# analysiscenter/pydens

Measured on NVIDIA H100. Metric: collocation points/sec (fit step), higher is better.
Workload: dtype f32

## Files before the change

__graft_entry__.py:

```python
import concurrent.futures
import os
import subprocess
import sys

ROOT = os.path.dirname(os.path.abspath(__file__))
CSRC = os.path.join(ROOT, 'pydens_b200', 'csrc')
BUILD = os.path.join(ROOT, 'build')
LIB = os.path.join(ROOT, 'pydens_b200', 'libpinn_b200.so')
EMUL_SRC = os.path.join(ROOT, 'tests', 'emul', 'pinn_emul.cpp')
EMUL_LIB = os.path.join(ROOT, 'tests', 'emul', 'libpinn_emul.so')

NVCC_FLAGS = ['-gencode', 'arch=compute_90a,code=sm_90a', '-lineinfo', '-O3', '-std=c++17',
              '-Xcompiler', '-fPIC', '-I', os.path.join(ROOT, 'include')]
UNITS = ([('step_gen', 4, 3, 4), ('step_gen', 4, 0, 2), ('step_gen', 3, 2, 3), ('step_gen', 3, 0, 1)]
         + [('step', n, 0, n) for n in (4, 3)]
         + [('step_gen', n, 0, n) for n in (2, 1, 0)] + [('step', n, 0, n) for n in (2, 1, 0)]
         + [('step_gmem', n, n, n) for n in (6, 5)] + [('hi_jet', n, 3, 4) for n in (4, 3, 2, 1)]
         + [('wide', n, 0, n) for n in (4, 3, 2, 1, 0)] + [('small', n, 0, n) for n in (4, 3, 2, 1, 0)])
HEADERS = ['pinn_device.cuh', 'pinn_step_kernel.cuh', 'pinn_wide_kernel.cuh', 'pinn_small_kernel.cuh', 'pinn_host_plan.h',
           'pinn_device_hi.cuh', 'pinn_hi_kernel.cuh', os.path.join(ROOT, 'include', 'pinn_b200.h')]


def _mtime(path):
    return os.path.getmtime(path) if os.path.exists(path) else 0.0


def _nvcc():
    for cand in (os.environ.get('NVCC'), '/usr/local/cuda/bin/nvcc', 'nvcc'):
        if cand and (os.path.isabs(cand) and os.path.exists(cand) or not os.path.isabs(cand)):
            return cand
    return 'nvcc'


def _compile_one(unit):
    if isinstance(unit, str):
        src, name, defines = unit, os.path.splitext(unit)[0], []
    else:
        family, nf, lo, hi = unit
        src, name = 'pinn_instances.cu', 'pinn_%s_nf%d_%d-%d' % (family, nf, lo, hi)
        defines = ['-DPINN_UNIT=PINN_%s' % family.upper(), '-DPINN_NF=%d' % nf, '-DPINN_LO=%d' % lo, '-DPINN_HI=%d' % hi]
    obj = os.path.join(BUILD, name + '.o')
    srcp = os.path.join(CSRC, src)
    newest = max([_mtime(srcp)] + [_mtime(h if os.path.isabs(h) else os.path.join(CSRC, h)) for h in HEADERS])
    if _mtime(obj) >= newest:
        return obj, ''
    cmd = [_nvcc()] + NVCC_FLAGS + defines + ['-Xptxas', '-v', '-c', srcp, '-o', obj]
    res = subprocess.run(cmd, capture_output=True, text=True)
    if res.returncode != 0:
        raise RuntimeError('nvcc failed for %s:\n%s\n%s' % (name, res.stdout, res.stderr))
    return obj, res.stderr


def build(verbose=False, force=False):
# ... 66 lines not shown
```

pydens_b200/csrc/pinn_device.cuh:

```cuda
#pragma once

#include <stdint.h>
#include <math.h>
#include "../../include/pinn_b200.h"

#if defined(__CUDACC__)
#define PINN_HD __host__ __device__ __forceinline__
#define PINN_D  __device__ __forceinline__
#else
#define PINN_HD inline
#define PINN_D  inline
struct float4 { float x, y, z, w; };
struct float2 { float x, y; };
inline float2 make_float2(float x, float y) { float2 r; r.x = x; r.y = y; return r; }
#endif

#ifndef PINN_UNR_WIDE
#define PINN_UNR_WIDE 4
#endif
#ifndef PINN_BWD_UNR_WIDE
#define PINN_BWD_UNR_WIDE 1
#endif

#define PINN_FFMA2(a2, s, c2) make_float2(fmaf((a2).x, (s), (c2).x), fmaf((a2).y, (s), (c2).y))
#define PINN_FMUL2(a2, s)     make_float2((a2).x * (s), (a2).y * (s))
#define PINN_FFMA2V(a2, b2, c2) make_float2(fmaf((a2).x, (b2).x, (c2).x), fmaf((a2).y, (b2).y, (c2).y))
#define PINN_FMUL2V(a2, b2)     make_float2((a2).x * (b2).x, (a2).y * (b2).y)

namespace pinn {

struct DevLayer {
    int n_in, n_out, act;
    int w_off, b_off;
    int wt_s;
    int w_s;
    int b_s;
    int n_out_p4, n_in_p8;
    int unit_base;
    int post_base;
// ... 221 lines not shown
    const float2 out = PINN_FFMA2(t, k.p, make_float2(k.r, k.r));
    return k.ident ? z : out;
}

PINN_HD ActD act_from_stored(const ActC& k, float a) {
    ActD r;
    if (k.zs) { act_terms_z(k.zs, a, r.a, r.s1, r.s2, r.s3); return r; }
    r.a = a;
    r.s1 = fmaf(fmaf(k.c2, a, k.c1), a, k.c0);
    r.s2 = r.s1 * fmaf(k.d1, a, k.d0);
    r.s3 = r.s1 * fmaf(fmaf(k.e2, a, k.e1), a, k.e0);
    return r;
}

template <int NF, int NS, bool GEN = true>
PINN_HD void load_post_jet(const float* __restrict__ row, int RS, const ActC& k, float (&a)[1 + NF + NS]) {
    float av = row[0];
    float s1 = fmaf(fmaf(k.c2, av, k.c1), av, k.c0);
    float s2 = s1 * fmaf(k.d1, av, k.d0);
    if (GEN && k.zs) { float s3; act_terms_z(k.zs, row[0], av, s1, s2, s3); }
    a[0] = av;
#pragma unroll
    for (int d = 0; d < NF; ++d) {
        float zd = row[(1 + d) * RS];
        a[1 + d] = s1 * zd;
        if (d < NS) {
            float zdd = row[(1 + NF + d) * RS];
            a[1 + NF + d] = fmaf(s2 * zd, zd, s1 * zdd);
        }
    }
}

template <int NF, int NS, bool GEN = true>
PINN_HD void load_post_jet2(const float* __restrict__ rowa, const float* __restrict__ rowb, int RS, const ActC& k,
                            float2 (&a)[1 + NF + NS]) {
    float2 av = make_float2(rowa[0], rowb[0]);
    float2 s1 = PINN_FFMA2V(PINN_FFMA2(av, k.c2, make_float2(k.c1, k.c1)), av, make_float2(k.c0, k.c0));
    float2 s2 = PINN_FMUL2V(s1, PINN_FFMA2(av, k.d1, make_float2(k.d0, k.d0)));
    if (GEN && k.zs) {
        float s3;
        const float za = av.x, zb = av.y;
        act_terms_z(k.zs, za, av.x, s1.x, s2.x, s3);
        act_terms_z(k.zs, zb, av.y, s1.y, s2.y, s3);
    }
    a[0] = av;
#pragma unroll
    for (int d = 0; d < NF; ++d) {
        const float2 zd = make_float2(rowa[(1 + d) * RS], rowb[(1 + d) * RS]);
        a[1 + d] = PINN_FMUL2V(s1, zd);
        if (d < NS) {
            const float2 zdd = make_float2(rowa[(1 + NF + d) * RS], rowb[(1 + NF + d) * RS]);
            a[1 + NF + d] = PINN_FFMA2V(PINN_FMUL2V(s2, zd), zd, PINN_FMUL2V(s1, zdd));
        }
    }
}

template <int NF, int NS, int NB, bool GEN = true>
PINN_HD void fwd_block_hidden(const float* __restrict__ Wt, int wt_stride, const float* __restrict__ bias,
                              int n_in, const float* __restrict__ in_rows, int RS, const ActC& in_act,
                              float2 (&acc)[NB * 2][1 + NF + NS]) {
    constexpr int C = 1 + NF + NS;
#pragma unroll
    for (int j = 0; j < NB * 2; ++j) {
        acc[j][0] = make_float2(bias[2 * j], bias[2 * j + 1]);
#pragma unroll
        for (int c = 1; c < C; ++c) acc[j][c] = make_float2(0.0f, 0.0f);
    }
    constexpr int UNR = (C >= 8) ? PINN_UNR_WIDE : ((C >= 6) ? 2 : 1);
#pragma unroll UNR
    for (int k = 0; k < n_in; ++k) {
        float a[C];
        load_post_jet<NF, NS, GEN>(in_rows + (size_t)k * C * RS, RS, in_act, a);
        const float4* wrow = reinterpret_cast<const float4*>(Wt + (size_t)k * wt_stride);
#pragma unroll
        for (int g = 0; g < NB; ++g) {
            const float4 w = wrow[g];
            const float2 w01 = make_float2(w.x, w.y), w23 = make_float2(w.z, w.w);
#pragma unroll
            for (int c = 0; c < C; ++c) {
                acc[2 * g + 0][c] = PINN_FFMA2(w01, a[c], acc[2 * g + 0][c]);
                acc[2 * g + 1][c] = PINN_FFMA2(w23, a[c], acc[2 * g + 1][c]);
            }
        }
    }
}

template <int NF, int NS, int NB>
PINN_HD void fwd_block_input(const float* __restrict__ Wt, int wt_stride, const float* __restrict__ bias,
                             int n_in, const float* __restrict__ coords, int RS, const float* __restrict__ dirv,
                             float2 (&acc)[NB * 2][1 + NF + NS]) {
    constexpr int C = 1 + NF + NS;
#pragma unroll
    for (int j = 0; j < NB * 2; ++j) {
        acc[j][0] = make_float2(bias[2 * j], bias[2 * j + 1]);
#pragma unroll
        for (int c = 1; c < C; ++c) acc[j][c] = make_float2(0.0f, 0.0f);
    }
#pragma unroll 1
    for (int k = 0; k < n_in; ++k) {
        float x = coords[(size_t)k * RS];
        float vd[NF > 0 ? NF : 1];
#pragma unroll
        for (int d = 0; d < NF; ++d) vd[d] = dirv[d * PINN_MAX_DIMS + k];
        const float4* wrow = reinterpret_cast<const float4*>(Wt + (size_t)k * wt_stride);
#pragma unroll
        for (int g = 0; g < NB; ++g) {
            const float4 w = wrow[g];
            const float2 w01 = make_float2(w.x, w.y), w23 = make_float2(w.z, w.w);
            acc[2 * g + 0][0] = PINN_FFMA2(w01, x, acc[2 * g + 0][0]);
            acc[2 * g + 1][0] = PINN_FFMA2(w23, x, acc[2 * g + 1][0]);
#pragma unroll
            for (int d = 0; d < NF; ++d) {
                acc[2 * g + 0][1 + d] = PINN_FFMA2(w01, vd[d], acc[2 * g + 0][1 + d]);
                acc[2 * g + 1][1 + d] = PINN_FFMA2(w23, vd[d], acc[2 * g + 1][1 + d]);
            }
        }
    }
}

template <int NF, int NS, int NB, bool GEN = true>
PINN_HD void store_block(float* __restrict__ out_rows, int RS, const ActC& act, int j0, int n_out,
                         const float2 (&acc)[NB * 2][1 + NF + NS]) {
    constexpr int C = 1 + NF + NS;
#pragma unroll
    for (int h = 0; h < NB * 2; ++h) {
        const float2 a = act_store2<GEN>(act, acc[h][0]);
#pragma unroll
        for (int q = 0; q < 2; ++q) {
            const int j = 2 * h + q;
            const bool ok = j0 + j < n_out;
            float* row = out_rows + (size_t)(ok ? j0 + j : j0) * C * RS;
            if (ok) row[0] = q ? a.y : a.x;
#pragma unroll
            for (int c = 1; c < C; ++c)
                if (ok) row[(size_t)c * RS] = q ? acc[h][c].y : acc[h][c].x;
        }
    }
}

template <int NF, int NS, int JF, bool GEN = true>
PINN_HD void fwd_layer(const DevLayer& L, const float* __restrict__ sw, const float* __restrict__ in_rows,
                       bool in_is_coords, int in_act_id, const float* __restrict__ dirv,
                       float* __restrict__ out_rows, int RS) {
    constexpr int NBMAX = JF / 4;
    const float* Wt = sw + L.wt_s;
    const float* bias = sw + L.b_s;
    const ActC in_act = make_actc(in_act_id);
    const ActC out_act = make_actc(L.act);
#pragma unroll 1
    for (int j0 = 0; j0 < L.n_out; j0 += JF) {
        int nb = (L.n_out_p4 - j0) / 4;
        if (nb > NBMAX) nb = NBMAX;
#define PINN_FWD_CASE(NB)                                                                           \
        {                                                                                           \
            float2 acc[NB * 2][1 + NF + NS];                                                        \
            if (in_is_coords)                                                                       \
                fwd_block_input<NF, NS, NB>(Wt + j0, L.n_out_p4, bias + j0, L.n_in, in_rows, RS,    \
                                            dirv, acc);                                             \
            else                                                                                    \
                fwd_block_hidden<NF, NS, NB, GEN>(Wt + j0, L.n_out_p4, bias + j0, L.n_in, in_rows, RS,   \
                                             in_act, acc);                                          \
            store_block<NF, NS, NB, GEN>(out_rows, RS, out_act, j0, L.n_out, acc);                    \
        }
        if (NBMAX >= 4 && nb == 4) PINN_FWD_CASE(4)
        else if (NBMAX >= 3 && nb == 3) PINN_FWD_CASE(3)
        else if (NBMAX >= 2 && nb == 2) PINN_FWD_CASE(2)
        else PINN_FWD_CASE(1)
#undef PINN_FWD_CASE
    }
}

template <bool GEN = true>
PINN_HD const float* layer_output(const DevPlan& P, int p, const float* __restrict__ units, int C, int RS,
                                  int& act_id) {
    const DevLayer& Lp = P.layer[p];
    if (GEN && Lp.post_base >= 0) { act_id = PINN_ACT_NONE; return units + (size_t)Lp.post_base * C * RS; }
    act_id = Lp.act;
    return units + (size_t)Lp.unit_base * C * RS;
}

template <int NF, int NS>
PINN_HD void skip_sum_pass(const DevPlan& P, int l, float* __restrict__ units, int RS) {
    constexpr int C = 1 + NF + NS;
    const DevLayer& L = P.layer[l];
    const ActC own = make_actc(L.act);
    int src_act;
    const float* src_rows = layer_output(P, L.skip_src, units, C, RS, src_act);
    const ActC srcc = make_actc(src_act);
    const float* pre_rows = units + (size_t)L.unit_base * C * RS;
    float* post_rows = units + (size_t)L.post_base * C * RS;
#pragma unroll 1
    for (int j = 0; j < L.n_out; ++j) {
        float a[C], b[C];
        load_post_jet<NF, NS>(pre_rows + (size_t)j * C * RS, RS, own, a);
        load_post_jet<NF, NS>(src_rows + (size_t)j * C * RS, RS, srcc, b);
#pragma unroll
        for (int c = 0; c < C; ++c) post_rows[((size_t)j * C + c) * RS] = a[c] + b[c];
    }
}

template <int NF, int NS, bool GEN = true>
PINN_HD void fwd_final(const DevLayer& L, const float* __restrict__ sw, const float* __restrict__ in_rows,
                       bool in_is_coords, int in_act_id, const float* __restrict__ dirv, int RS,
                       float (&N)[1 + NF + NS]) {
    constexpr int C = 1 + NF + NS;
    const ActC in_act = make_actc(in_act_id);
    const float* w = sw + L.w_s;
    N[0] = sw[L.b_s];
#pragma unroll
    for (int c = 1; c < C; ++c) N[c] = 0.0f;
    if (in_is_coords) {
        for (int k = 0; k < L.n_in; ++k) {
            N[0] = fmaf(w[k], in_rows[(size_t)k * RS], N[0]);
#pragma unroll
            for (int d = 0; d < NF; ++d) N[1 + d] = fmaf(w[k], dirv[d * PINN_MAX_DIMS + k], N[1 + d]);
        }
    } else {
#pragma unroll 1
        for (int k = 0; k < L.n_in; ++k) {
            float a[C];
            load_post_jet<NF, NS, GEN>(in_rows + (size_t)k * C * RS, RS, in_act, a);
            float wk = w[k];
#pragma unroll
            for (int c = 0; c < C; ++c) N[c] = fmaf(wk, a[c], N[c]);
        }
    }
}

PINN_HD float powi_f(float x, int e) {
    bool neg = e < 0;
    unsigned n = neg ? (unsigned)(-e) : (unsigned)e;
    float r = 1.0f, b = x;
    while (n) { if (n & 1u) r *= b; b *= b; n >>= 1; }
    return neg ? 1.0f / r : r;
}

PINN_HD void eval_prog(const PinnInstr* __restrict__ prog, int n, float* __restrict__ scr, int RS,
                       const float* __restrict__ coords, const float* __restrict__ pvals,
                       const int* __restrict__ var_off) {
    for (int i = 0; i < n; ++i) {
        PinnInstr in = prog[i];
        float r;
        switch (in.op) {
            case PINN_OP_CONST: r = in.imm; break;
            case PINN_OP_COORD: r = coords[(size_t)in.a * RS]; break;
            case PINN_OP_VAR:   r = pvals[var_off[in.a]]; break;
            default: {
                float x = scr[(size_t)in.a * RS];
                switch (in.op) {
                    case PINN_OP_ADD:  r = x + scr[(size_t)in.b * RS]; break;
                    case PINN_OP_SUB:  r = x - scr[(size_t)in.b * RS]; break;
                    case PINN_OP_MUL:  r = x * scr[(size_t)in.b * RS]; break;
                    case PINN_OP_DIV:  r = x / scr[(size_t)in.b * RS]; break;
                    case PINN_OP_POW:  r = powf(x, scr[(size_t)in.b * RS]); break;
// ... 176 lines not shown
            Nb[1 + d] = nd;
        }
        Nb[0] = nb0;
    } else {
        Nb[0] = vb;
#pragma unroll
        for (int d = 0; d < NF; ++d) { Nb[1 + d] = vdb[d]; if (d < NS) Nb[1 + NF + d] = vddb[d]; }
    }
    return sbar;
}

template <int NF, int NS>
PINN_HD void act_adjoint(const ActD& f, const float (&pre)[1 + NF + NS], const float (&ab)[1 + NF + NS],
                         float (&zb)[1 + NF + NS]) {
    float z0 = f.s1 * ab[0];
#pragma unroll
    for (int d = 0; d < NF; ++d) {
        float zd = pre[1 + d];
        float t = f.s2 * zd;
        z0 = fmaf(t, ab[1 + d], z0);
        float zdb = f.s1 * ab[1 + d];
        if (d < NS) {
            float q = ab[1 + NF + d];
            zdb = fmaf(2.0f * t, q, zdb);
            z0 = fmaf(fmaf(f.s3 * zd, zd, f.s2 * pre[1 + NF + d]), q, z0);
            zb[1 + NF + d] = f.s1 * q;
        }
        zb[1 + d] = zdb;
    }
    zb[0] = z0;
}

template <int NF, int NS, bool GEN = true>
PINN_HD void act_adjoint2(const ActC& k, const float2 (&pre)[1 + NF + NS], const float2 (&ab)[1 + NF + NS],
                          float2 (&zb)[1 + NF + NS]) {
    const float2 a = pre[0];
    float2 s1 = PINN_FFMA2V(PINN_FFMA2(a, k.c2, make_float2(k.c1, k.c1)), a, make_float2(k.c0, k.c0));
    float2 s2 = PINN_FMUL2V(s1, PINN_FFMA2(a, k.d1, make_float2(k.d0, k.d0)));
    float2 s3 = PINN_FMUL2V(s1, PINN_FFMA2V(PINN_FFMA2(a, k.e2, make_float2(k.e1, k.e1)), a, make_float2(k.e0, k.e0)));
    if (GEN && k.zs) {
        float av;
        act_terms_z(k.zs, a.x, av, s1.x, s2.x, s3.x);
        act_terms_z(k.zs, a.y, av, s1.y, s2.y, s3.y);
    }
    float2 z0 = PINN_FMUL2V(s1, ab[0]);
#pragma unroll
    for (int d = 0; d < NF; ++d) {
        const float2 zd = pre[1 + d];
        const float2 t = PINN_FMUL2V(s2, zd);
        z0 = PINN_FFMA2V(t, ab[1 + d], z0);
        float2 zdb = PINN_FMUL2V(s1, ab[1 + d]);
        if (d < NS) {
            const float2 q = ab[1 + NF + d];
            zdb = PINN_FFMA2V(PINN_FMUL2(t, 2.0f), q, zdb);
            const float2 w = PINN_FFMA2V(PINN_FMUL2V(s3, zd), zd, PINN_FMUL2V(s2, pre[1 + NF + d]));
            z0 = PINN_FFMA2V(w, q, z0);
            zb[1 + NF + d] = PINN_FMUL2V(s1, q);
        }
        zb[1 + d] = zdb;
    }
    zb[0] = z0;
}

#if defined(__CUDA_ARCH__)
template <int S, int NV>
__device__ __forceinline__ void warp_transpose_stage(float (&v)[NV], int lane) {
    if constexpr (S >= NV) {
#pragma unroll
        for (int i = 0; i < NV; ++i) v[i] += __shfl_xor_sync(0xffffffffu, v[i], S);
    } else {
        const bool up = (lane & S) != 0;
#pragma unroll
        for (int i = 0; i < S; ++i) {
            const float lo = v[i], hi = v[i + S];
            const float send = up ? lo : hi;
            const float keep = up ? hi : lo;
            v[i] = keep + __shfl_xor_sync(0xffffffffu, send, S);
// ... 24 lines not shown
struct GradSink {
    float* wacc;
    int dump;
#if !defined(__CUDACC__)
    bool atomic;
#endif
    PINN_HD void add_if(bool valid, int idx, float val) const {
#if defined(__CUDA_ARCH__)
        const int i = valid ? idx : dump; wacc[i] += val;
#else
        if (valid) wacc[idx] += val;
#endif
    }
    PINN_HD void add(int idx, float val) const { wacc[idx] += val; }
};

template <int NF, int NS>
PINN_HD void bias_grad(const DevLayer& L, const float* __restrict__ out_rows, int RS, const GradSink& sink) {
    constexpr int C = 1 + NF + NS;
#pragma unroll 1
    for (int j0 = 0; j0 < L.n_out; j0 += 32) {
        float v[32];
#pragma unroll
        for (int i = 0; i < 32; ++i) {
            const int j = j0 + i < L.n_out ? j0 + i : L.n_out - 1;
            v[i] = out_rows[(size_t)j * C * RS];
        }
        emit_entries<32>(v, [&](int e, float t) {
            sink.add_if(j0 + e < L.n_out, L.b_off + j0 + e, t);
        });
    }
}

template <int NF, int NS, int JJ, bool SKIP, bool GEN = SKIP>
PINN_HD void bwd_layer(const DevLayer& L, int below_act_id, const float* __restrict__ sw,
                       const float* __restrict__ out_rows, float* __restrict__ in_rows, int RS,
                       const GradSink& sink,
                       const float* __restrict__ load_rows, int load_act_id,
                       const float* __restrict__ adj_in ,
                       float* __restrict__ adj_out ,
                       float* __restrict__ dump_rows ) {
    constexpr int C = 1 + NF + NS;
    constexpr int JB = 8;
    const float* W = sw + L.w_s;
    const ActC below = make_actc(below_act_id);
    const ActC load_act = make_actc(SKIP ? load_act_id : below_act_id);
    if (!SKIP) load_rows = in_rows;
    const bool fold_bias = (L.n_in & (JB - 1)) != 0;
    const int n_cols = L.n_in + (fold_bias ? 1 : 0);
#pragma unroll 1
    for (int m0 = 0; m0 < n_cols; m0 += JB) {
        float2 post[JB / 2][C];
#pragma unroll
        for (int h = 0; h < JB / 2; ++h) {
            const int ma = m0 + 2 * h, mb = ma + 1;
            const int ca = ma < L.n_in ? ma : L.n_in - 1, cb = mb < L.n_in ? mb : L.n_in - 1;
            load_post_jet2<NF, NS, GEN>(load_rows + (size_t)ca * C * RS, load_rows + (size_t)cb * C * RS, RS, load_act,
                                   post[h]);
            if (ma == L.n_in) {
                post[h][0].x = 1.0f;
#pragma unroll
                for (int c = 1; c < C; ++c) post[h][c].x = 0.0f;
            }
            if (mb == L.n_in) {
                post[h][0].y = 1.0f;
#pragma unroll
                for (int c = 1; c < C; ++c) post[h][c].y = 0.0f;
            }
        }
        float2 acc[JB / 2][C];
#pragma unroll
        for (int h = 0; h < JB / 2; ++h)
#pragma unroll
            for (int c = 0; c < C; ++c) acc[h][c] = make_float2(0.0f, 0.0f);
        if (SKIP && adj_in) {
#pragma unroll
            for (int h = 0; h < JB / 2; ++h) {
                const int ma = m0 + 2 * h < L.n_in ? m0 + 2 * h : L.n_in - 1;
                const int mb = m0 + 2 * h + 1 < L.n_in ? m0 + 2 * h + 1 : L.n_in - 1;
#pragma unroll
                for (int c = 0; c < C; ++c)
                    acc[h][c] = make_float2(adj_in[((size_t)ma * C + c) * RS], adj_in[((size_t)mb * C + c) * RS]);
            }
        }

        constexpr int BUNR = (C >= 8) ? PINN_BWD_UNR_WIDE : 1;
#pragma unroll BUNR
        for (int j0 = 0; j0 < L.n_out; j0 += JJ) {
            float v[JJ * JB];
#pragma unroll
            for (int jj = 0; jj < JJ; ++jj) {
                const int j = j0 + jj;
                const int jc = j < L.n_out ? j : L.n_out - 1;
                const float* row = out_rows + (size_t)jc * C * RS;
                float zb[C];
#pragma unroll
                for (int c = 0; c < C; ++c) zb[c] = row[(size_t)c * RS];
                const float4* wrow = reinterpret_cast<const float4*>(W + (size_t)j * L.n_in_p8 + m0);
                const float4 w0 = wrow[0], w1 = wrow[1];
                const float2 w[JB / 2] = {make_float2(w0.x, w0.y), make_float2(w0.z, w0.w),
                                          make_float2(w1.x, w1.y), make_float2(w1.z, w1.w)};
#pragma unroll
                for (int h = 0; h < JB / 2; ++h) {
                    float2 e = PINN_FMUL2(post[h][0], zb[0]);
#pragma unroll
                    for (int c = 0; c < C; ++c) {
                        acc[h][c] = PINN_FFMA2(w[h], zb[c], acc[h][c]);
                        if (c > 0) e = PINN_FFMA2(post[h][c], zb[c], e);
                    }
                    v[jj * JB + 2 * h] = e.x;
                    v[jj * JB + 2 * h + 1] = e.y;
                }
            }
            emit_entries<JJ * JB>(v, [&](int e, float t) {
                const int j = j0 + e / JB, m = m0 + e % JB;
                sink.add_if(j < L.n_out && m <= L.n_in, m < L.n_in ? L.w_off + j * L.n_in + m : L.b_off + j, t);
            });
        }
#pragma unroll
        for (int h = 0; h < JB / 2; ++h) {
            const bool oka = m0 + 2 * h < L.n_in, okb = m0 + 2 * h + 1 < L.n_in;
            const float* rowa = in_rows + (size_t)(oka ? m0 + 2 * h : 0) * C * RS;
            const float* rowb = in_rows + (size_t)(okb ? m0 + 2 * h + 1 : 0) * C * RS;
            float2 pre[C], zb[C];
#pragma unroll
            for (int c = 0; c < C; ++c) pre[c] = make_float2(rowa[(size_t)c * RS], rowb[(size_t)c * RS]);
            act_adjoint2<NF, NS, GEN>(below, pre, acc[h], zb);
            float* wa = oka ? in_rows + (size_t)(m0 + 2 * h) * C * RS : dump_rows;
            float* wb = okb ? in_rows + (size_t)(m0 + 2 * h + 1) * C * RS : dump_rows;
#pragma unroll
            for (int c = 0; c < C; ++c) { wa[(size_t)c * RS] = zb[c].x; wb[(size_t)c * RS] = zb[c].y; }
            if (SKIP && adj_out) {
                float* sa = adj_out + (size_t)(oka ? m0 + 2 * h : 0) * C * RS;
                float* sb = adj_out + (size_t)(okb ? m0 + 2 * h + 1 : 0) * C * RS;
#pragma unroll
                for (int c = 0; c < C; ++c) {
                    if (oka) sa[(size_t)c * RS] = acc[h][c].x;
                    if (okb) sb[(size_t)c * RS] = acc[h][c].y;
                }
            }
        }
    }
    if (!fold_bias) bias_grad<NF, NS>(L, out_rows, RS, sink);
}

template <int NF, int NS>
PINN_HD void wgrad_input_layer(const DevLayer& L, const float* __restrict__ out_rows,
                               const float* __restrict__ coords, int RS, const float* __restrict__ dirv,
                               const GradSink& sink) {
    constexpr int C = 1 + NF + NS;
    float2 x[PINN_MAX_DIMS / 2];
    float2 dv[NF > 0 ? NF : 1][PINN_MAX_DIMS / 2];
#pragma unroll
    for (int h = 0; h < PINN_MAX_DIMS / 2; ++h) {
        const int ma = 2 * h, mb = 2 * h + 1;
        x[h] = make_float2((ma < L.n_in) ? coords[(size_t)ma * RS] : (ma == L.n_in ? 1.0f : 0.0f),
                           (mb < L.n_in) ? coords[(size_t)mb * RS] : (mb == L.n_in ? 1.0f : 0.0f));
#pragma unroll
        for (int d = 0; d < NF; ++d) dv[d][h] = make_float2(dirv[d * PINN_MAX_DIMS + ma], dirv[d * PINN_MAX_DIMS + mb]);
    }
#pragma unroll 1
    for (int j0 = 0; j0 < L.n_out; j0 += 4) {
        float v[4 * PINN_MAX_DIMS];
#pragma unroll
        for (int jj = 0; jj < 4; ++jj) {
            const int j = j0 + jj < L.n_out ? j0 + jj : L.n_out - 1;
            const float* row = out_rows + (size_t)j * C * RS;
            float zb[1 + NF];
#pragma unroll
            for (int c = 0; c < 1 + NF; ++c) zb[c] = row[(size_t)c * RS];
#pragma unroll
            for (int h = 0; h < PINN_MAX_DIMS / 2; ++h) {
                float2 e = PINN_FMUL2(x[h], zb[0]);
#pragma unroll
                for (int d = 0; d < NF; ++d) e = PINN_FFMA2(dv[d][h], zb[1 + d], e);
                v[jj * PINN_MAX_DIMS + 2 * h] = e.x;
                v[jj * PINN_MAX_DIMS + 2 * h + 1] = e.y;
            }
        }
        emit_entries<4 * PINN_MAX_DIMS>(v, [&](int e, float t) {
            const int j = j0 + e / PINN_MAX_DIMS, m = e % PINN_MAX_DIMS;
            sink.add_if(j < L.n_out && m <= L.n_in && m < PINN_MAX_DIMS,
                        m < L.n_in ? L.w_off + j * L.n_in + m : L.b_off + j, t);
        });
    }
    if (L.n_in >= PINN_MAX_DIMS) bias_grad<NF, NS>(L, out_rows, RS, sink);
}

template <int NF, int NS>
struct PointPartials { float loss, sbar, vbar[PINN_MAX_VARS]; };

template <int NF, int NS, int JF, bool GEN = true>
PINN_HD float point_step(const DevPlan& P, const float* __restrict__ sw ,
                         const float* __restrict__ pvals ,
                         float* __restrict__ st, int RS, bool valid, float inv_n,
                         const GradSink& sink, PointPartials<NF, NS>& part) {
    constexpr int C = 1 + NF + NS;
    const int Ln = P.n_layers;
    float* coords = st;
    float* units = st + (size_t)P.row_units * RS;
    float* scr = st + (size_t)P.row_scr * RS;

#pragma unroll 1
    for (int l = 0; l + 1 < Ln; ++l) {
        const DevLayer& L = P.layer[l];
        int in_act = PINN_ACT_NONE;
        const float* in_rows = (l == 0) ? coords : layer_output<GEN>(P, l - 1, units, C, RS, in_act);
        fwd_layer<NF, NS, JF, GEN>(L, sw, in_rows, l == 0, in_act, &P.dir_vec[0][0],
                                   units + (size_t)L.unit_base * C * RS, RS);
        if (GEN && L.skip_src >= 0) skip_sum_pass<NF, NS>(P, l, units, RS);
    }
    float N[C];
    {
        const DevLayer& L = P.layer[Ln - 1];
        int in_act = PINN_ACT_NONE;
        const float* in_rows = (Ln == 1) ? coords : layer_output<GEN>(P, Ln - 2, units, C, RS, in_act);
        fwd_final<NF, NS, GEN>(L, sw, in_rows, Ln == 1, in_act, &P.dir_vec[0][0], RS, N);
    }

    float icj[C];
#pragma unroll
    for (int c = 0; c < C; ++c) icj[c] = 0.0f;
    if (P.has_ic) {
        eval_prog(P.ic, P.n_ic, scr, RS, coords, pvals, P.var_off);
#pragma unroll
// ... 15 lines not shown
#pragma unroll
    for (int i = 0; i < PINN_MAX_VARS; ++i)
        if (i < P.n_vars) part.vbar[i] = fmaf(rb, scr[(size_t)P.eq_out[1 + C + i] * RS], part.vbar[i]);
    if (GEN && P.ic_has_vars) {
#pragma unroll
        for (int i = 0; i < PINN_MAX_VARS; ++i) {
            if (i < P.n_vars) {
#pragma unroll
                for (int c = 0; c < C; ++c)
                    part.vbar[i] = fmaf(ub[c], scr[(size_t)P.ic_out[C * (1 + i) + c] * RS], part.vbar[i]);
            }
        }
    }

    float Nb[C];
    part.sbar += ansatz_adjoint<NF, NS>(P, as, ub, Nb);

    {
        const DevLayer& L = P.layer[Ln - 1];
        float* out_rows = units + (size_t)L.unit_base * C * RS;
#pragma unroll
        for (int c = 0; c < C; ++c) out_rows[(size_t)c * RS] = Nb[c];
    }
#pragma unroll 1
    for (int l = Ln - 1; l >= 1; --l) {
        const DevLayer& L = P.layer[l];
        float* out_rows = units + (size_t)L.unit_base * C * RS;
        const DevLayer& B = P.layer[l - 1];
        float* in_rows = units + (size_t)B.unit_base * C * RS;
        int load_act;
        const float* load_rows = layer_output<GEN>(P, l - 1, units, C, RS, load_act);
        const float* adj_in = B.adj_from >= 0 ? units + (size_t)P.layer[B.adj_from].post_base * C * RS : nullptr;
        float* adj_out = B.skip_src >= 0 ? units + (size_t)B.post_base * C * RS : nullptr;
        if (GEN && (B.post_base >= 0 || B.adj_from >= 0)) {
            if (L.n_out == 1) bwd_layer<NF, NS, 1, true>(L, B.act, sw, out_rows, in_rows, RS, sink, load_rows, load_act, adj_in, adj_out, scr);
            else              bwd_layer<NF, NS, 4, true>(L, B.act, sw, out_rows, in_rows, RS, sink, load_rows, load_act, adj_in, adj_out, scr);
        } else {
            if (L.n_out == 1) bwd_layer<NF, NS, 1, false, GEN>(L, B.act, sw, out_rows, in_rows, RS, sink, in_rows, B.act, nullptr, nullptr, scr);
            else              bwd_layer<NF, NS, 4, false, GEN>(L, B.act, sw, out_rows, in_rows, RS, sink, in_rows, B.act, nullptr, nullptr, scr);
        }
    }
    {
        const DevLayer& L = P.layer[0];
        float* out_rows = units + (size_t)L.unit_base * C * RS;
        wgrad_input_layer<NF, NS>(L, out_rows, coords, RS, &P.dir_vec[0][0], sink);
    }
    return r;
}

template <int JF>
PINN_HD float point_forward(const DevPlan& P, const float* __restrict__ sw, const float* __restrict__ pvals,
                            float* __restrict__ st, int RS, int row_scr_fwd) {
    const int Ln = P.n_layers;
    float* coords = st;
    float* units = st + (size_t)P.row_units * RS;
    float* scr = st + (size_t)row_scr_fwd * RS;
    float dummy_dir[1] = {0.0f};
    for (int l = 0; l + 1 < Ln; ++l) {
        const DevLayer& L = P.layer[l];
        int in_act = PINN_ACT_NONE;
        const float* in_rows = (l == 0) ? coords : layer_output(P, l - 1, units, 1, RS, in_act);
        fwd_layer<0, 0, JF>(L, sw, in_rows, l == 0, in_act, dummy_dir, units + (size_t)L.unit_base * RS, RS);
        if (L.skip_src >= 0) skip_sum_pass<0, 0>(P, l, units, RS);
    }
    float N[1];
    {
        const DevLayer& L = P.layer[Ln - 1];
        int in_act = PINN_ACT_NONE;
        const float* in_rows = (Ln == 1) ? coords : layer_output(P, Ln - 2, units, 1, RS, in_act);
        fwd_final<0, 0>(L, sw, in_rows, Ln == 1, in_act, dummy_dir, RS, N);
    }
    float icj[1] = {0.0f};
// ... 12 lines not shown
```

pydens_b200/csrc/pinn_step_kernel.cuh:

```cuda
#pragma once

#include <cuda_runtime.h>
#include <stdint.h>
#include "pinn_device.cuh"

#ifndef PINN_COMM_MAX_RANKS
#define PINN_COMM_MAX_RANKS 8
#endif

namespace pinn {

constexpr int RS = 32;

struct StepArgs {
    const float* params;
    const float* points;
    uint64_t seed;
    const uint64_t* step_ptr;
    uint64_t step_val;
    uint64_t point_offset;
    long long n_points;
    float inv_n;
    float* out;
    float* residual;
// ... 364 lines not shown
    stage_weights(smem, SL, P, a.params);
    const float* sw = smem + SL.weights_f;
    float* wacc_all = warp_accumulators(a, smem, SL, n_out_floats, nwarps);

    GradSink sink;
    sink.wacc = wacc_all + warp * n_out_floats;
    sink.dump = P.n_params + 2;

    const long long gw = (long long)blockIdx.x * nwarps + warp;
    const long long total_warps = (long long)gridDim.x * nwarps;
    float* st = (GMEM ? a.spill + (size_t)gw * a.rows_total * RS : smem + SL.storage_f + (size_t)warp * a.rows_total * RS) + lane;

    const uint64_t step = a.step_ptr ? *a.step_ptr : a.step_val;
    const long long n_tiles = (a.n_points + 31) / 32;
    PointPartials<NF, NS> part;
    part.loss = 0.0f; part.sbar = 0.0f;
#pragma unroll
    for (int i = 0; i < PINN_MAX_VARS; ++i) part.vbar[i] = 0.0f;

    for (long long tile = (long long)warp * gridDim.x + blockIdx.x; tile < n_tiles; tile += total_warps) {
        const long long pl = tile * 32 + lane;
        const bool valid = pl < a.n_points;
        const long long pe = valid ? pl : a.n_points - 1;
        if (a.points) {
            const float* src = a.points + (size_t)pe * P.total;
            for (int k = 0; k < P.total; ++k) st[k * RS] = __ldg(src + k);
        } else {
            const uint64_t gidx = a.point_offset + (uint64_t)pe;
            Philox4 b0 = philox_block(gidx, step, a.seed, 0u);
            Philox4 b1 = b0;
            if (P.total > 4) b1 = philox_block(gidx, step, a.seed, 1u);
            for (int k = 0; k < P.total; ++k) st[k * RS] = sample_column(P.cols[k], k, gidx, step, a.seed, b0, b1);
        }
        float r = point_step<NF, NS, JF, GEN>(P, sw, a.params, st, RS, valid, a.inv_n, sink, part);
        if (a.residual && valid) a.residual[pl] = r;
    }

    {
        float v = warp_sum(part.loss);
        if (lane == 0) sink.add(P.n_params, v);
        v = warp_sum(part.sbar);
        if (lane == 0) sink.add(P.log_scale_off, v);
#pragma unroll
        for (int i = 0; i < PINN_MAX_VARS; ++i) {
            if (i < P.n_vars) {
                float t = warp_sum(part.vbar[i]);
                if (lane == 0) sink.add(P.var_off[i], t);
            }
        }
    }
    __syncthreads();

    cta_partial(a, wacc_all, n_out_floats, nwarps);
    finish_grid(a, n_out_floats);
}


struct MultiArgs {
    float* params;
    float* exp_avg;
    float* exp_avg_sq;
    const float* mask;
    float* step_tensors;
    int n_step_tensors;
    const float* points;
    uint64_t seed;
    unsigned long long* step_counter;
// ... 138 lines not shown
```

pydens_b200/csrc/pinn_wide_kernel.cuh:

```cuda
#pragma once

#include "pinn_step_kernel.cuh"

namespace pinn {
namespace wide {

constexpr int T = 128;
constexpr int NT_MAX = 512;
constexpr int KW = 64;
constexpr int MAX_LAYERS = 6;
constexpr int LDS = KW + 4;
constexpr int LXB = T + 4;

constexpr int S_W = 0;
constexpr int S_A = S_W + KW * LDS * 4;
constexpr int S_GB = S_A + T * LDS * 4;
constexpr int S_D = S_GB + T * LDS * 4;
constexpr int S_X = S_D + T * LDS * 4;
constexpr int S_XB = S_X + 24 * T * 4;
constexpr int S_WACC = S_XB + 16 * LXB * 4;
constexpr int S_SMALL1 = S_WACC + (MAX_LAYERS - 2) * KW * KW * 4;
constexpr int S_OUT = S_SMALL1 + KW * 16 * 4;
constexpr int S_SMALLH = S_OUT + KW * 8 * 4;
constexpr int S_MISC = S_SMALLH + (MAX_LAYERS - 2) * KW * 8 * 4;
constexpr int MISC_FLOATS = 1536;
constexpr int SMEM_BYTES = S_MISC + MISC_FLOATS * 4;
constexpr int ACC_FLOATS = (S_MISC - S_WACC) / 4;
static_assert(SMEM_BYTES <= 227 * 1024, "shared memory of one CTA");

constexpr int M_BIAS = 0;
constexpr int M_W0 = M_BIAS + MAX_LAYERS * 64;
constexpr int M_WD = M_W0 + 64 * 8;
constexpr int M_WOUT = M_WD + PINN_MAX_DIRS * 64;
constexpr int M_SCAL = M_WOUT + 64;
constexpr int M_END = M_SCAL + 8 * (NT_MAX / 32);
static_assert(M_END <= MISC_FLOATS, "misc area");

__device__ __forceinline__ void split_tf32(float x, uint32_t& hi, uint32_t& lo) {
    asm("cvt.rna.tf32.f32 %0, %1;" : "=r"(hi) : "f"(x));
    asm("cvt.rna.tf32.f32 %0, %1;" : "=r"(lo) : "f"(x - __uint_as_float(hi)));
}
__device__ __forceinline__ float tf32_rn(float x) {
    uint32_t r;
    asm("cvt.rna.tf32.f32 %0, %1;" : "=r"(r) : "f"(x));
    return __uint_as_float(r);
}
__device__ __forceinline__ void mma_tf32(float (&d)[4], const uint32_t (&a)[4], uint32_t b0, uint32_t b1) {
    asm volatile("mma.sync.aligned.m16n8k8.row.col.f32.tf32.tf32.f32 {%0,%1,%2,%3}, {%4,%5,%6,%7}, {%8,%9}, {%0,%1,%2,%3};"
                 : "+f"(d[0]), "+f"(d[1]), "+f"(d[2]), "+f"(d[3])
                 : "r"(a[0]), "r"(a[1]), "r"(a[2]), "r"(a[3]), "r"(b0), "r"(b1));
}
__device__ __forceinline__ void mma3(float (&d)[4], const uint32_t (&ah)[4], const uint32_t (&al)[4],
                                     uint32_t bh0, uint32_t bh1, uint32_t bl0, uint32_t bl1) {
    mma_tf32(d, al, bh0, bh1);
    mma_tf32(d, ah, bl0, bl1);
    mma_tf32(d, ah, bh0, bh1);
}

__device__ __forceinline__ void ld8(const float* __restrict__ blk, int k0, float (&v)[8]) {
    const float* q = blk + (size_t)(k0 >> 2) * (T * 4);
    const float4 a = *reinterpret_cast<const float4*>(q), b = *reinterpret_cast<const float4*>(q + T * 4);
    v[0] = a.x; v[1] = a.y; v[2] = a.z; v[3] = a.w; v[4] = b.x; v[5] = b.y; v[6] = b.z; v[7] = b.w;
}
__device__ __forceinline__ void st8(float* __restrict__ blk, int k0, const float (&v)[8]) {
    float* q = blk + (size_t)(k0 >> 2) * (T * 4);
    *reinterpret_cast<float4*>(q) = make_float4(v[0], v[1], v[2], v[3]);
    *reinterpret_cast<float4*>(q + T * 4) = make_float4(v[4], v[5], v[6], v[7]);
}
__device__ __forceinline__ void st_row8(uint8_t* base, int p, int k0, const float (&v)[8]) {
    float* q = reinterpret_cast<float*>(base) + p * LDS + k0;
    *reinterpret_cast<float4*>(q) = make_float4(v[0], v[1], v[2], v[3]);
    *reinterpret_cast<float4*>(q + 4) = make_float4(v[4], v[5], v[6], v[7]);
}
__device__ __forceinline__ void ld_row8(const uint8_t* base, int p, int k0, float (&v)[8]) {
    const float* q = reinterpret_cast<const float*>(base) + p * LDS + k0;
    const float4 a = *reinterpret_cast<const float4*>(q), b = *reinterpret_cast<const float4*>(q + 4);
    v[0] = a.x; v[1] = a.y; v[2] = a.z; v[3] = a.w; v[4] = b.x; v[5] = b.y; v[6] = b.z; v[7] = b.w;
}

__host__ __device__ inline int rup(int x, int m) { return (x + m - 1) / m * m; }
__host__ __device__ inline size_t spill_floats_per_cta(int n_layers, int C) {
    const int upper = n_layers - 2 > 0 ? n_layers - 2 : 0;
    return (size_t)(1 + upper * C) * T * KW;
}

__device__ __forceinline__ void stage_layer(uint8_t* smem, const float* __restrict__ params, const DevLayer& L, bool transpose) {
    float* w_s = reinterpret_cast<float*>(smem + S_W);
    for (int i = threadIdx.x; i < KW * KW; i += blockDim.x) {
        const int n = i >> 6, k = i & 63;
// ... 560 lines not shown
```

Baseline: 947.5 million.

## Compute per-layer weight gradients with 3xTF32 tensor-core MMA in step kernel

Adds a warp-level wgrad_tc routine that forms each layer's weight and bias gradients as a reduction over points and jet channels. It uses split-TF32 mma.sync (three MMAs per tile to keep roughly FP32 accuracy), replacing the per-thread FMA outer-product accumulation in bwd_layer, which gains a flag to skip its gradient work. Forward layers now store post-activation jets rather than pre-activation values, so loads no longer recompute the activation derivatives, and the adjoint is reformulated to take the stored jet. This relies on points being laid out contiguously across lanes. It costs extra conversion and MMA instructions, plus a changed storage convention, and the old path is kept for the general-activation and gmem cases.

```diff
diff --git a/__graft_entry__.py b/__graft_entry__.py
--- a/__graft_entry__.py
+++ b/__graft_entry__.py
@@ -17,8 +17,8 @@
          + [('step_gen', n, 0, n) for n in (2, 1, 0)] + [('step', n, 0, n) for n in (2, 1, 0)]
          + [('step_gmem', n, n, n) for n in (6, 5)] + [('hi_jet', n, 3, 4) for n in (4, 3, 2, 1)]
          + [('wide', n, 0, n) for n in (4, 3, 2, 1, 0)] + [('small', n, 0, n) for n in (4, 3, 2, 1, 0)])
-HEADERS = ['pinn_device.cuh', 'pinn_step_kernel.cuh', 'pinn_wide_kernel.cuh', 'pinn_small_kernel.cuh', 'pinn_host_plan.h',
-           'pinn_device_hi.cuh', 'pinn_hi_kernel.cuh', os.path.join(ROOT, 'include', 'pinn_b200.h')]
+HEADERS = ['pinn_device.cuh', 'pinn_mma.cuh', 'pinn_step_kernel.cuh', 'pinn_wide_kernel.cuh', 'pinn_small_kernel.cuh',
+           'pinn_host_plan.h', 'pinn_device_hi.cuh', 'pinn_hi_kernel.cuh', os.path.join(ROOT, 'include', 'pinn_b200.h')]
 
 
 def _mtime(path):
diff --git a/pydens_b200/csrc/pinn_device.cuh b/pydens_b200/csrc/pinn_device.cuh
--- a/pydens_b200/csrc/pinn_device.cuh
+++ b/pydens_b200/csrc/pinn_device.cuh
@@ -5,6 +5,7 @@
 #include "../../include/pinn_b200.h"
 
 #if defined(__CUDACC__)
+#include "pinn_mma.cuh"
 #define PINN_HD __host__ __device__ __forceinline__
 #define PINN_D  __device__ __forceinline__
 #else
@@ -292,27 +293,26 @@
 }
 
 template <int NF, int NS, bool GEN = true>
-PINN_HD void load_post_jet2(const float* __restrict__ rowa, const float* __restrict__ rowb, int RS, const ActC& k,
-                            float2 (&a)[1 + NF + NS]) {
-    float2 av = make_float2(rowa[0], rowb[0]);
-    float2 s1 = PINN_FFMA2V(PINN_FFMA2(av, k.c2, make_float2(k.c1, k.c1)), av, make_float2(k.c0, k.c0));
-    float2 s2 = PINN_FMUL2V(s1, PINN_FFMA2(av, k.d1, make_float2(k.d0, k.d0)));
+PINN_HD void load_jet(const float* __restrict__ row, int RS, const ActC& k, float (&a)[1 + NF + NS]) {
+    if (GEN && k.zs) { load_post_jet<NF, NS, GEN>(row, RS, k, a); return; }
+#pragma unroll
+    for (int c = 0; c < 1 + NF + NS; ++c) a[c] = row[(size_t)c * RS];
+}
+
+template <int NF, int NS, bool GEN = true>
+PINN_HD void load_jet2(const float* __restrict__ rowa, const float* __restrict__ rowb, int RS, const ActC& k,
+                       float2 (&a)[1 + NF + NS]) {
+    constexpr int C = 1 + NF + NS;
     if (GEN && k.zs) {
-        float s3;
-        const float za = av.x, zb = av.y;
-        act_terms_z(k.zs, za, av.x, s1.x, s2.x, s3);
-        act_terms_z(k.zs, zb, av.y, s1.y, s2.y, s3);
-    }
-    a[0] = av;
-#pragma unroll
-    for (int d = 0; d < NF; ++d) {
-        const float2 zd = make_float2(rowa[(1 + d) * RS], rowb[(1 + d) * RS]);
-        a[1 + d] = PINN_FMUL2V(s1, zd);
-        if (d < NS) {
-            const float2 zdd = make_float2(rowa[(1 + NF + d) * RS], rowb[(1 + NF + d) * RS]);
-            a[1 + NF + d] = PINN_FFMA2V(PINN_FMUL2V(s2, zd), zd, PINN_FMUL2V(s1, zdd));
-        }
-    }
+        float pa[C], pb[C];
+        load_post_jet<NF, NS, GEN>(rowa, RS, k, pa);
+        load_post_jet<NF, NS, GEN>(rowb, RS, k, pb);
+#pragma unroll
+        for (int c = 0; c < C; ++c) a[c] = make_float2(pa[c], pb[c]);
+        return;
+    }
+#pragma unroll
+    for (int c = 0; c < C; ++c) a[c] = make_float2(rowa[(size_t)c * RS], rowb[(size_t)c * RS]);
 }
 
 template <int NF, int NS, int NB, bool GEN = true>
@@ -330,7 +330,7 @@
 #pragma unroll UNR
     for (int k = 0; k < n_in; ++k) {
         float a[C];
-        load_post_jet<NF, NS, GEN>(in_rows + (size_t)k * C * RS, RS, in_act, a);
+        load_jet<NF, NS, GEN>(in_rows + (size_t)k * C * RS, RS, in_act, a);
         const float4* wrow = reinterpret_cast<const float4*>(Wt + (size_t)k * wt_stride);
 #pragma unroll
         for (int g = 0; g < NB; ++g) {
@@ -385,15 +385,28 @@
 #pragma unroll
     for (int h = 0; h < NB * 2; ++h) {
         const float2 a = act_store2<GEN>(act, acc[h][0]);
+        float2 post[C];
+        post[0] = a;
+        const float2 s1 = PINN_FFMA2V(PINN_FFMA2(a, act.c2, make_float2(act.c1, act.c1)), a, make_float2(act.c0, act.c0));
+        const float2 s2 = PINN_FMUL2V(s1, PINN_FFMA2(a, act.d1, make_float2(act.d0, act.d0)));
+#pragma unroll
+        for (int d = 0; d < NF; ++d) {
+            const float2 zd = acc[h][1 + d];
+            post[1 + d] = PINN_FMUL2V(s1, zd);
+            if (d < NS) post[1 + NF + d] = PINN_FFMA2V(PINN_FMUL2V(s2, zd), zd, PINN_FMUL2V(s1, acc[h][1 + NF + d]));
+        }
+        if (GEN && act.zs) {
+#pragma unroll
+            for (int c = 1; c < C; ++c) post[c] = acc[h][c];
+        }
 #pragma unroll
         for (int q = 0; q < 2; ++q) {
             const int j = 2 * h + q;
             const bool ok = j0 + j < n_out;
             float* row = out_rows + (size_t)(ok ? j0 + j : j0) * C * RS;
-            if (ok) row[0] = q ? a.y : a.x;
-#pragma unroll
-            for (int c = 1; c < C; ++c)
-                if (ok) row[(size_t)c * RS] = q ? acc[h][c].y : acc[h][c].x;
+#pragma unroll
+            for (int c = 0; c < C; ++c)
+                if (ok) row[(size_t)c * RS] = q ? post[c].y : post[c].x;
         }
     }
 }
@@ -452,8 +465,8 @@
 #pragma unroll 1
     for (int j = 0; j < L.n_out; ++j) {
         float a[C], b[C];
-        load_post_jet<NF, NS>(pre_rows + (size_t)j * C * RS, RS, own, a);
-        load_post_jet<NF, NS>(src_rows + (size_t)j * C * RS, RS, srcc, b);
+        load_jet<NF, NS>(pre_rows + (size_t)j * C * RS, RS, own, a);
+        load_jet<NF, NS>(src_rows + (size_t)j * C * RS, RS, srcc, b);
 #pragma unroll
         for (int c = 0; c < C; ++c) post_rows[((size_t)j * C + c) * RS] = a[c] + b[c];
     }
@@ -479,7 +492,7 @@
 #pragma unroll 1
         for (int k = 0; k < L.n_in; ++k) {
             float a[C];
-            load_post_jet<NF, NS, GEN>(in_rows + (size_t)k * C * RS, RS, in_act, a);
+            load_jet<NF, NS, GEN>(in_rows + (size_t)k * C * RS, RS, in_act, a);
             float wk = w[k];
 #pragma unroll
             for (int c = 0; c < C; ++c) N[c] = fmaf(wk, a[c], N[c]);
@@ -722,17 +735,36 @@
 }
 
 template <int NF, int NS, bool GEN = true>
-PINN_HD void act_adjoint2(const ActC& k, const float2 (&pre)[1 + NF + NS], const float2 (&ab)[1 + NF + NS],
+PINN_HD void act_adjoint2(const ActC& k, const float2 (&jet)[1 + NF + NS], const float2 (&ab)[1 + NF + NS],
                           float2 (&zb)[1 + NF + NS]) {
-    const float2 a = pre[0];
-    float2 s1 = PINN_FFMA2V(PINN_FFMA2(a, k.c2, make_float2(k.c1, k.c1)), a, make_float2(k.c0, k.c0));
-    float2 s2 = PINN_FMUL2V(s1, PINN_FFMA2(a, k.d1, make_float2(k.d0, k.d0)));
-    float2 s3 = PINN_FMUL2V(s1, PINN_FFMA2V(PINN_FFMA2(a, k.e2, make_float2(k.e1, k.e1)), a, make_float2(k.e0, k.e0)));
-    if (GEN && k.zs) {
-        float av;
-        act_terms_z(k.zs, a.x, av, s1.x, s2.x, s3.x);
-        act_terms_z(k.zs, a.y, av, s1.y, s2.y, s3.y);
-    }
+    const float2 a = jet[0];
+    if (!(GEN && k.zs)) {
+        const float2 s1 = PINN_FFMA2V(PINN_FFMA2(a, k.c2, make_float2(k.c1, k.c1)), a, make_float2(k.c0, k.c0));
+        const float2 k1 = PINN_FFMA2(a, k.d1, make_float2(k.d0, k.d0));
+        float2 z0 = PINN_FMUL2V(s1, ab[0]);
+#pragma unroll
+        for (int d = 0; d < NF; ++d) {
+            const float2 ad = jet[1 + d];
+            const float2 t = PINN_FMUL2V(k1, ad);
+            z0 = PINN_FFMA2V(t, ab[1 + d], z0);
+            float2 zdb = PINN_FMUL2V(s1, ab[1 + d]);
+            if (d < NS) {
+                const float2 q = ab[1 + NF + d];
+                zdb = PINN_FFMA2V(PINN_FMUL2(t, 2.0f), q, zdb);
+                const float2 w = PINN_FFMA2V(PINN_FMUL2(ad, k.d1), ad, PINN_FMUL2V(k1, jet[1 + NF + d]));
+                z0 = PINN_FFMA2V(w, q, z0);
+                zb[1 + NF + d] = PINN_FMUL2V(s1, q);
+            }
+            zb[1 + d] = zdb;
+        }
+        zb[0] = z0;
+        return;
+    }
+    const float2* pre = jet;
+    float2 s1, s2, s3;
+    float av;
+    act_terms_z(k.zs, a.x, av, s1.x, s2.x, s3.x);
+    act_terms_z(k.zs, a.y, av, s1.y, s2.y, s3.y);
     float2 z0 = PINN_FMUL2V(s1, ab[0]);
 #pragma unroll
     for (int d = 0; d < NF; ++d) {
@@ -823,7 +855,81 @@
     }
 }
 
-template <int NF, int NS, int JJ, bool SKIP, bool GEN = SKIP>
+template <int NF, int NS>
+PINN_HD void wgrad_tc(const DevLayer& L, const float* __restrict__ out_rows, const float* __restrict__ post_rows,
+                      int RS, const GradSink& sink) {
+    constexpr int C = 1 + NF + NS;
+#if defined(__CUDA_ARCH__)
+    const int lane = threadIdx.x & 31, g = lane >> 2, t = lane & 3;
+    const float* zt = out_rows - lane + 4 * t;
+    const float* pt = post_rows - lane + 4 * t;
+    __syncwarp();
+#pragma unroll 1
+    for (int j0 = 0; j0 < L.n_out; j0 += 16) {
+        const int ja = min(j0 + g, L.n_out - 1), jb = min(j0 + g + 8, L.n_out - 1);
+        const float* ra = zt + (size_t)ja * C * RS;
+        const float* rb = zt + (size_t)jb * C * RS;
+#pragma unroll 1
+        for (int m0 = 0; m0 <= L.n_in; m0 += 16) {
+            const int ma = m0 + g, mb = m0 + 8 + g;
+            const bool bias_a = ma == L.n_in, bias_b = mb == L.n_in;
+            const float* rn[2] = {pt + (size_t)min(ma, L.n_in - 1) * C * RS, pt + (size_t)min(mb, L.n_in - 1) * C * RS};
+            float acc[2][4] = {{0.0f, 0.0f, 0.0f, 0.0f}, {0.0f, 0.0f, 0.0f, 0.0f}};
+            constexpr int CHU = C >= 4 ? 2 : 1;
+#pragma unroll CHU
+            for (int ch = 0; ch < 2 * C; ++ch) {
+                const int c = ch >> 1;
+                const int off = c * RS + 16 * (ch & 1);
+                const float4 a0 = *reinterpret_cast<const float4*>(ra + off);
+                const float4 a1 = *reinterpret_cast<const float4*>(rb + off);
+                float4 b[2] = {*reinterpret_cast<const float4*>(rn[0] + off), *reinterpret_cast<const float4*>(rn[1] + off)};
+                const float one = c == 0 ? 1.0f : 0.0f;
+                if (bias_a) b[0] = make_float4(one, one, one, one);
+                if (bias_b) b[1] = make_float4(one, one, one, one);
+#pragma unroll
+                for (int s = 0; s < 2; ++s) {
+                    uint32_t ah[4], al[4];
+                    split_tf32(s ? a0.z : a0.x, ah[0], al[0]);
+                    split_tf32(s ? a1.z : a1.x, ah[1], al[1]);
+                    split_tf32(s ? a0.w : a0.y, ah[2], al[2]);
+                    split_tf32(s ? a1.w : a1.y, ah[3], al[3]);
+#pragma unroll
+                    for (int nt = 0; nt < 2; ++nt) {
+                        uint32_t bh0, bl0, bh1, bl1;
+                        split_tf32(s ? b[nt].z : b[nt].x, bh0, bl0);
+                        split_tf32(s ? b[nt].w : b[nt].y, bh1, bl1);
+                        mma3(acc[nt], ah, al, bh0, bh1, bl0, bl1);
+                    }
+                }
+            }
+#pragma unroll
+            for (int nt = 0; nt < 2; ++nt)
+#pragma unroll
+                for (int r = 0; r < 4; ++r) {
+                    const int j = j0 + g + 8 * (r >> 1), m = m0 + 8 * nt + 2 * t + (r & 1);
+                    sink.add_if(j < L.n_out && m <= L.n_in, m < L.n_in ? L.w_off + j * L.n_in + m : L.b_off + j, acc[nt][r]);
+                }
+        }
+    }
+    __syncwarp();
+#else
+    for (int j = 0; j < L.n_out; ++j) {
+        const float* zr = out_rows + (size_t)j * C * RS;
+        for (int m = 0; m <= L.n_in; ++m) {
+            float e;
+            if (m == L.n_in) e = zr[0];
+            else {
+                const float* pr = post_rows + (size_t)m * C * RS;
+                e = 0.0f;
+                for (int c = 0; c < C; ++c) e = fmaf(zr[(size_t)c * RS], pr[(size_t)c * RS], e);
+            }
+            sink.add(m < L.n_in ? L.w_off + j * L.n_in + m : L.b_off + j, e);
+        }
+    }
+#endif
+}
+
+template <int NF, int NS, int JJ, bool SKIP, bool GEN = SKIP, bool WG = true>
 PINN_HD void bwd_layer(const DevLayer& L, int below_act_id, const float* __restrict__ sw,
                        const float* __restrict__ out_rows, float* __restrict__ in_rows, int RS,
                        const GradSink& sink,
@@ -840,13 +946,13 @@
     const bool fold_bias = (L.n_in & (JB - 1)) != 0;
     const int n_cols = L.n_in + (fold_bias ? 1 : 0);
 #pragma unroll 1
-    for (int m0 = 0; m0 < n_cols; m0 += JB) {
+    for (int m0 = 0; m0 < (WG ? n_cols : L.n_in); m0 += JB) {
         float2 post[JB / 2][C];
 #pragma unroll
-        for (int h = 0; h < JB / 2; ++h) {
+        for (int h = 0; h < (WG ? JB / 2 : 0); ++h) {
             const int ma = m0 + 2 * h, mb = ma + 1;
             const int ca = ma < L.n_in ? ma : L.n_in - 1, cb = mb < L.n_in ? mb : L.n_in - 1;
-            load_post_jet2<NF, NS, GEN>(load_rows + (size_t)ca * C * RS, load_rows + (size_t)cb * C * RS, RS, load_act,
+            load_jet2<NF, NS, GEN>(load_rows + (size_t)ca * C * RS, load_rows + (size_t)cb * C * RS, RS, load_act,
                                    post[h]);
             if (ma == L.n_in) {
                 post[h][0].x = 1.0f;
@@ -893,17 +999,18 @@
                                           make_float2(w1.x, w1.y), make_float2(w1.z, w1.w)};
 #pragma unroll
                 for (int h = 0; h < JB / 2; ++h) {
-                    float2 e = PINN_FMUL2(post[h][0], zb[0]);
-#pragma unroll
-                    for (int c = 0; c < C; ++c) {
-                        acc[h][c] = PINN_FFMA2(w[h], zb[c], acc[h][c]);
-                        if (c > 0) e = PINN_FFMA2(post[h][c], zb[c], e);
+#pragma unroll
+                    for (int c = 0; c < C; ++c) acc[h][c] = PINN_FFMA2(w[h], zb[c], acc[h][c]);
+                    if (WG) {
+                        float2 e = PINN_FMUL2(post[h][0], zb[0]);
+#pragma unroll
+                        for (int c = 1; c < C; ++c) e = PINN_FFMA2(post[h][c], zb[c], e);
+                        v[jj * JB + 2 * h] = e.x;
+                        v[jj * JB + 2 * h + 1] = e.y;
                     }
-                    v[jj * JB + 2 * h] = e.x;
-                    v[jj * JB + 2 * h + 1] = e.y;
                 }
             }
-            emit_entries<JJ * JB>(v, [&](int e, float t) {
+            if (WG) emit_entries<JJ * JB>(v, [&](int e, float t) {
                 const int j = j0 + e / JB, m = m0 + e % JB;
                 sink.add_if(j < L.n_out && m <= L.n_in, m < L.n_in ? L.w_off + j * L.n_in + m : L.b_off + j, t);
             });
@@ -932,7 +1039,7 @@
             }
         }
     }
-    if (!fold_bias) bias_grad<NF, NS>(L, out_rows, RS, sink);
+    if (WG && !fold_bias) bias_grad<NF, NS>(L, out_rows, RS, sink);
 }
 
 template <int NF, int NS>
@@ -981,7 +1088,7 @@
 template <int NF, int NS>
 struct PointPartials { float loss, sbar, vbar[PINN_MAX_VARS]; };
 
-template <int NF, int NS, int JF, bool GEN = true>
+template <int NF, int NS, int JF, bool GEN = true, bool TC = true>
 PINN_HD float point_step(const DevPlan& P, const float* __restrict__ sw ,
                          const float* __restrict__ pvals ,
                          float* __restrict__ st, int RS, bool valid, float inv_n,
@@ -1063,12 +1170,16 @@
         const float* load_rows = layer_output<GEN>(P, l - 1, units, C, RS, load_act);
         const float* adj_in = B.adj_from >= 0 ? units + (size_t)P.layer[B.adj_from].post_base * C * RS : nullptr;
         float* adj_out = B.skip_src >= 0 ? units + (size_t)B.post_base * C * RS : nullptr;
+        const bool tc = TC && L.n_out > 1 && !(GEN && make_actc(load_act).zs);
+        if (tc) wgrad_tc<NF, NS>(L, out_rows, load_rows, RS, sink);
         if (GEN && (B.post_base >= 0 || B.adj_from >= 0)) {
             if (L.n_out == 1) bwd_layer<NF, NS, 1, true>(L, B.act, sw, out_rows, in_rows, RS, sink, load_rows, load_act, adj_in, adj_out, scr);
+            else if (tc)      bwd_layer<NF, NS, 4, true, true, false>(L, B.act, sw, out_rows, in_rows, RS, sink, load_rows, load_act, adj_in, adj_out, scr);
             else              bwd_layer<NF, NS, 4, true>(L, B.act, sw, out_rows, in_rows, RS, sink, load_rows, load_act, adj_in, adj_out, scr);
         } else {
-            if (L.n_out == 1) bwd_layer<NF, NS, 1, false, GEN>(L, B.act, sw, out_rows, in_rows, RS, sink, in_rows, B.act, nullptr, nullptr, scr);
-            else              bwd_layer<NF, NS, 4, false, GEN>(L, B.act, sw, out_rows, in_rows, RS, sink, in_rows, B.act, nullptr, nullptr, scr);
+            if (L.n_out == 1)   bwd_layer<NF, NS, 1, false, GEN>(L, B.act, sw, out_rows, in_rows, RS, sink, in_rows, B.act, nullptr, nullptr, scr);
+            else if ((TC && !GEN) || tc) bwd_layer<NF, NS, 4, false, GEN, false>(L, B.act, sw, out_rows, in_rows, RS, sink, in_rows, B.act, nullptr, nullptr, scr);
+            else                bwd_layer<NF, NS, 4, false, GEN>(L, B.act, sw, out_rows, in_rows, RS, sink, in_rows, B.act, nullptr, nullptr, scr);
         }
     }
     {
diff --git a/pydens_b200/csrc/pinn_mma.cuh b/pydens_b200/csrc/pinn_mma.cuh
--- /dev/null
+++ b/pydens_b200/csrc/pinn_mma.cuh
@@ -0,0 +1,23 @@
+#pragma once
+
+#include <stdint.h>
+
+namespace pinn {
+
+__device__ __forceinline__ void split_tf32(float x, uint32_t& hi, uint32_t& lo) {
+    asm("cvt.rna.tf32.f32 %0, %1;" : "=r"(hi) : "f"(x));
+    asm("cvt.rna.tf32.f32 %0, %1;" : "=r"(lo) : "f"(x - __uint_as_float(hi)));
+}
+__device__ __forceinline__ void mma_tf32(float (&d)[4], const uint32_t (&a)[4], uint32_t b0, uint32_t b1) {
+    asm volatile("mma.sync.aligned.m16n8k8.row.col.f32.tf32.tf32.f32 {%0,%1,%2,%3}, {%4,%5,%6,%7}, {%8,%9}, {%0,%1,%2,%3};"
+                 : "+f"(d[0]), "+f"(d[1]), "+f"(d[2]), "+f"(d[3])
+                 : "r"(a[0]), "r"(a[1]), "r"(a[2]), "r"(a[3]), "r"(b0), "r"(b1));
+}
+__device__ __forceinline__ void mma3(float (&d)[4], const uint32_t (&ah)[4], const uint32_t (&al)[4],
+                                     uint32_t bh0, uint32_t bh1, uint32_t bl0, uint32_t bl1) {
+    mma_tf32(d, al, bh0, bh1);
+    mma_tf32(d, ah, bl0, bl1);
+    mma_tf32(d, ah, bh0, bh1);
+}
+
+}
diff --git a/pydens_b200/csrc/pinn_step_kernel.cuh b/pydens_b200/csrc/pinn_step_kernel.cuh
--- a/pydens_b200/csrc/pinn_step_kernel.cuh
+++ b/pydens_b200/csrc/pinn_step_kernel.cuh
@@ -420,7 +420,7 @@
             if (P.total > 4) b1 = philox_block(gidx, step, a.seed, 1u);
             for (int k = 0; k < P.total; ++k) st[k * RS] = sample_column(P.cols[k], k, gidx, step, a.seed, b0, b1);
         }
-        float r = point_step<NF, NS, JF, GEN>(P, sw, a.params, st, RS, valid, a.inv_n, sink, part);
+        float r = point_step<NF, NS, JF, GEN, !GMEM>(P, sw, a.params, st, RS, valid, a.inv_n, sink, part);
         if (a.residual && valid) a.residual[pl] = r;
     }
 
diff --git a/pydens_b200/csrc/pinn_wide_kernel.cuh b/pydens_b200/csrc/pinn_wide_kernel.cuh
--- a/pydens_b200/csrc/pinn_wide_kernel.cuh
+++ b/pydens_b200/csrc/pinn_wide_kernel.cuh
@@ -36,25 +36,10 @@
 constexpr int M_END = M_SCAL + 8 * (NT_MAX / 32);
 static_assert(M_END <= MISC_FLOATS, "misc area");
 
-__device__ __forceinline__ void split_tf32(float x, uint32_t& hi, uint32_t& lo) {
-    asm("cvt.rna.tf32.f32 %0, %1;" : "=r"(hi) : "f"(x));
-    asm("cvt.rna.tf32.f32 %0, %1;" : "=r"(lo) : "f"(x - __uint_as_float(hi)));
-}
 __device__ __forceinline__ float tf32_rn(float x) {
     uint32_t r;
     asm("cvt.rna.tf32.f32 %0, %1;" : "=r"(r) : "f"(x));
     return __uint_as_float(r);
-}
-__device__ __forceinline__ void mma_tf32(float (&d)[4], const uint32_t (&a)[4], uint32_t b0, uint32_t b1) {
-    asm volatile("mma.sync.aligned.m16n8k8.row.col.f32.tf32.tf32.f32 {%0,%1,%2,%3}, {%4,%5,%6,%7}, {%8,%9}, {%0,%1,%2,%3};"
-                 : "+f"(d[0]), "+f"(d[1]), "+f"(d[2]), "+f"(d[3])
-                 : "r"(a[0]), "r"(a[1]), "r"(a[2]), "r"(a[3]), "r"(b0), "r"(b1));
-}
-__device__ __forceinline__ void mma3(float (&d)[4], const uint32_t (&ah)[4], const uint32_t (&al)[4],
-                                     uint32_t bh0, uint32_t bh1, uint32_t bl0, uint32_t bl1) {
-    mma_tf32(d, al, bh0, bh1);
-    mma_tf32(d, ah, bl0, bl1);
-    mma_tf32(d, ah, bh0, bh1);
 }
 
 __device__ __forceinline__ void ld8(const float* __restrict__ blk, int k0, float (&v)[8]) {
```

New measurement: 959.5 million (median of 6 runs). 1.3% higher.
